# robertteleng/aria-slam

Measured on AMD Instinct MI355X. Metric: frames/s ORB extract+BF-match, 640x480 @2000 kp, higher is better.
Workload: dtype u8

## Files before the change

### aria_slam_amd/csrc/fast_blur_stream.hip

```cpp
#include <hip/hip_runtime.h>

#include <algorithm>
#include <cstdint>
#include <cstdio>
#include <cstdlib>

#include "common.h"
#include "orb_device.h"
#include "orb_kernels.h"

namespace aria {

namespace {

constexpr int kRing = 16;
#ifndef ARIA_STREAM_PEND_LDS
#define ARIA_STREAM_PEND_LDS 1
#endif
constexpr int kQ1 = 256;
constexpr int kQ2 = 512;
#ifndef ARIA_STREAM_COMPACT_LDS
#define ARIA_STREAM_COMPACT_LDS 1
#endif
#if ARIA_STREAM_COMPACT_LDS
// ... 776 lines not shown
                const uint8_t* rowb = s_rawb + roff(rb);
                const bool reuse = oy == hprev_row;
                uint32_t qb0[4], qb1[4], qa0[4] = {0, 0, 0, 0}, qa1[4] = {0, 0, 0, 0};
#pragma unroll
                for (int i = 0; i < 4; i++) {
                    const uint32_t* qb = reinterpret_cast<const uint32_t*>(rowb + xo[i]);
                    qb0[i] = qb[0]; qb1[i] = qb[1];
                }
                if (!reuse) {
#pragma unroll
                    for (int i = 0; i < 4; i++) {
                        const uint32_t* qa = reinterpret_cast<const uint32_t*>(rowa + xo[i]);
                        qa0[i] = qa[0]; qa1[i] = qa[1];
                    }
                }
                uint32_t outw = 0;
#pragma unroll
                for (int i = 0; i < 4; i++) {
                    const us2v wx = __builtin_bit_cast(us2v, xw[i]);
                    uint32_t h0 = hprev[i];
                    if (!reuse) h0 = __builtin_amdgcn_udot2(__builtin_bit_cast(us2v, __builtin_amdgcn_perm(qa1[i], qa0[i], xs[i])), wx, 0u, false);
                    const uint32_t bot = __builtin_amdgcn_perm(qb1[i], qb0[i], xs[i]);
                    const uint32_t h1 = __builtin_amdgcn_udot2(__builtin_bit_cast(us2v, bot), wx, 0u, false);
                    const uint32_t v = __builtin_amdgcn_udot2(__builtin_bit_cast(us2v, h0 | (h1 << 16)), __builtin_bit_cast(us2v, cyp), 32768u, false);
                    outw = __builtin_amdgcn_perm(v, outw, put[i]);
                    hprev[i] = h1;
                }
                gstore_sv<uint32_t>(next0 + (int64_t)dy_next * A.next_pitch, nout_off, outw);
            }
            hprev_row = rb;
            dy_next++;
        }
        wave_sync();
    };
    for (int gi = 0; gi < G; gi += 2) {
        group(b0, gi);
        group(b1, gi + 1);
    }
}

#ifndef ARIA_STREAM_WAVES4
#define ARIA_STREAM_WAVES4 1
#endif
#if ARIA_STREAM_WAVES4
static_assert(ARIA_STREAM_COMPACT_LDS, "four waves per SIMD need the 10 240-byte LDS layout");
#define ARIA_STREAM_OCC __attribute__((amdgpu_waves_per_eu(4, 4)))
#else
#define ARIA_STREAM_OCC
#endif
template <int WPB>
__global__ __launch_bounds__(64 * WPB) ARIA_STREAM_OCC void k_fast_blur_stream(StreamArgs A, unsigned long long* __restrict__ stamps) {
    extern __shared__ __attribute__((aligned(16))) uint8_t smem[];
    const int lane = threadIdx.x & 63;
    const int wv = __builtin_amdgcn_readfirstlane((int)(threadIdx.x >> 6));
    const int w = A.w, h = A.h;
    const int D = (w + 3) >> 2, U = D + 2;
    int wave_id = (int)blockIdx.x * WPB + wv;
    bool role_pyr = false;
    if (ARIA_STREAM_SPLIT && A.next != nullptr) {
        role_pyr = (((wave_id >> 3) ^ __popc(wave_id >> 4)) & 1) != 0;
        wave_id = ((wave_id >> 4) << 3) | (wave_id & 7);
    }
    const int per_seg = 8 * A.panels8;
    const int seg = wave_id / per_seg, rr = wave_id - seg * per_seg;
    const int pw = (rr & 7) * A.panels8 + (rr >> 3);
    if (seg >= A.n_seg || pw >= A.panels) return;
    const int64_t total = (int64_t)A.n_frames * U;
    const int64_t pos0 = (int64_t)pw * kOwned - 1;
    int64_t pos = pos0 + lane;
    const bool valid = pos >= 0 && pos < total;
    pos = min(max(pos, (int64_t)0), total - 1);
    LaneRole R;
    R.frame = (int)(pos / U);
    const int j = (int)(pos - (int64_t)R.frame * U);
    R.gdw = j - 1;
    const int frame0 = __builtin_amdgcn_readfirstlane(R.frame);
    const int r4 = w & 3;
    if (R.gdw < 0 || R.gdw >= D) R.sel = 0x00010203u;
    else if (r4 && R.gdw == D - 1) R.sel = r4 == 1 ? 0x00010203u : r4 == 2 ? 0x01020302u : 0x02030201u;
    else R.sel = 0x03020100u;
    const bool data = valid && R.gdw >= 0 && R.gdw < D;
    R.owner = data && lane >= 1 && lane <= kOwned;
    const bool level_has_kp = (w > 2 * kEdgeThreshold) && (h > 2 * kEdgeThreshold);
    const int fx0 = kEdgeThreshold - 1, fx1 = w - kEdgeThreshold;
    R.xm0 = R.xm1 = 0;
    R.tailbits = 0;
    if (data) {
        const int x = 4 * R.gdw;
#pragma unroll
        for (int i = 0; i < 4; i++) {
            const bool scored = (lane >= 1 && lane <= kOwned) || (lane == 0 && i == 3) || (lane == 63 && i == 0);
            if (level_has_kp && scored && x + i >= fx0 && x + i <= fx1) {
                if (i < 2) R.xm0 |= (i & 1) ? 0x80000000u : 0x00008000u;
                else R.xm1 |= (i & 1) ? 0x80000000u : 0x00008000u;
            }
            if (x + i >= A.tail_start) R.tailbits |= 1u << i;
        }
    }
    uint8_t* wl = smem + wv * kWaveLds;
    const bool any_tail = __builtin_amdgcn_ballot_w64(R.tailbits != 0) != 0;
#if ARIA_STREAM_SPLIT
#ifdef ARIA_PROBE_SPLIT_EMPTY_PYR
    if (role_pyr) return;
#endif
    if (role_pyr) pyramid_wave(A, wl, lane, R, frame0, seg);
    else if (any_tail) stream_wave<WPB, true, true, false>(A, wl, lane, R, frame0, seg, stamps);
    else stream_wave<WPB, false, true, false>(A, wl, lane, R, frame0, seg, stamps);
#else
    (void)role_pyr;
#if ARIA_STREAM_PYR_INWALK
    if (A.next == nullptr) {
        if (any_tail) stream_wave<WPB, true, true, false>(A, wl, lane, R, frame0, seg, stamps);
        else stream_wave<WPB, false, true, false>(A, wl, lane, R, frame0, seg, stamps);
        return;
    }
#endif
    if (any_tail) stream_wave<WPB, true, true, true>(A, wl, lane, R, frame0, seg, stamps);
    else stream_wave<WPB, false, true, true>(A, wl, lane, R, frame0, seg, stamps);
#endif
}

bool stream_eligible(const Plan& P, const FrameSrc& S) {
    (void)S;
    for (int l = 0; l < kLevels; l++)
        if (P.lv[l].w < 16 || P.lv[l].h < 16) return false;
    return P.stream_ok != 0;
}

int stream_set_attributes() {
    ARIA_HIP(hipFuncSetAttribute(reinterpret_cast<const void*>(k_fast_blur_stream<1>), hipFuncAttributeMaxDynamicSharedMemorySize, 160 * 1024 - 64));
    ARIA_HIP(hipFuncSetAttribute(reinterpret_cast<const void*>(k_fast_blur_stream<2>), hipFuncAttributeMaxDynamicSharedMemorySize, 160 * 1024 - 64));
    ARIA_HIP(hipFuncSetAttribute(reinterpret_cast<const void*>(k_fast_blur_stream<4>), hipFuncAttributeMaxDynamicSharedMemorySize, 160 * 1024 - 64));
    return ARIA_OK;
}

int blur_tail_start(int tie_mode, int w) {
    switch (tie_mode) {
        case 0: return 0;
        case 2: return w & ~7;
        case 3: return w & ~15;
        default: return w & ~3;
    }
}

void launch_fast_blur_stream(const Plan& P, const FrameSrc& S, const DeviceScratch& D, int n_frames, hipStream_t st,
                             Profiler* prof, LaunchCtx& ctx) {
#ifdef ARIA_DIAG
    static const bool want_stamps = [] { const char* e = aria_getenv("ARIA_STREAM_STAMPS"); return e && e[0] == '1'; }();
#else
    const bool want_stamps = false;
#endif
    static unsigned long long* d_stamps = nullptr;
    if (want_stamps && !d_stamps) hipMalloc(&d_stamps, 8 * sizeof(unsigned long long));
    (void)ctx;
    static const int seg_force = [] { const char* e = aria_getenv("ARIA_STREAM_SEG_ROWS"); return e ? atoi(e) : 0; }();
    static const int wpb = [] { const char* e = aria_getenv("ARIA_STREAM_WPB"); const int v = e ? atoi(e) : 1; return (v == 2 || v == 4) ? v : 1; }();
    for (int l = 0; l < kLevels; l++) {
        const LevelGeom& g = P.lv[l];
        const int U = ((g.w + 3) >> 2) + 2;
        const int64_t total = (int64_t)n_frames * U;
        const int64_t panels = (total + kOwned - 1) / kOwned;
        int n_seg = (int)std::min<int64_t>(std::max<int64_t>((6 * 256 * 12 + panels - 1) / panels, 1), std::max(g.h / 64, 1));
        if (seg_force > 0) n_seg = std::min(std::max(g.h / seg_force, 1), 64);
        const int seg_rows = ((g.h + n_seg - 1) / n_seg + 3) & ~3;
        n_seg = (g.h + seg_rows - 1) / seg_rows;
        const int64_t panels8 = (panels + 7) / 8;
        const int64_t waves = 8 * panels8 * n_seg * ((ARIA_STREAM_SPLIT && l + 1 < kLevels) ? 2 : 1);
        const dim3 grid((unsigned)((waves + wpb - 1) / wpb));
        StreamArgs A{};
        A.seg_rows = seg_rows; A.n_seg = n_seg; A.panels = (int)panels; A.panels8 = (int)panels8;
        if (l == 0) { A.src = S.img; A.src_fstride = S.frame_stride; A.src_pitch = S.row_stride; }
        else { A.src = D.raw + g.raw_off; A.src_fstride = P.raw_frame_bytes; A.src_pitch = g.pitch; }
        A.blur = D.blur + g.blur_off; A.blur_fstride = P.blur_frame_bytes; A.blur_pitch = g.pitch;
        A.cand = D.cand + g.cand_off; A.cand_fstride = P.cand_frame_entries; A.cand_cap = g.cand_cap;
        A.cand_cnt = D.cand_cnt + l; A.err = D.err;
        A.w = g.w; A.h = g.h; A.n_frames = n_frames; A.thr = P.fast_threshold; A.tail_start = blur_tail_start(P.tie_mode, g.w);
        if (l + 1 < kLevels) {
            const LevelGeom& gn = P.lv[l + 1];
            A.next = D.raw + gn.raw_off; A.next_fstride = P.raw_frame_bytes; A.next_pitch = gn.pitch; A.next_w = gn.w; A.next_h = gn.h;
            A.xt = D.tab + gn.xtab; A.yt = D.tab + gn.ytab; A.xinv = D.tab + gn.xinv; A.ytr = D.tab + gn.ytr;
        } else {
            A.ytr = D.tab + P.lv[1].ytr;
        }
        static const size_t lds_pad = [] { const char* e = aria_getenv("ARIA_STREAM_LDS_KB"); return e ? (size_t)atoi(e) * 1024 : (size_t)0; }();
#define ARIA_FS_LAUNCH(N) ARIA_LAUNCH(prof, (k_fast_blur_stream<N>), grid, dim3(64 * N), std::max((size_t)N * kWaveLds, lds_pad), st, A, d_stamps)
        if (d_stamps) hipMemsetAsync(d_stamps, 0, 8 * sizeof(unsigned long long), st);
        if (wpb == 1) ARIA_FS_LAUNCH(1); else if (wpb == 2) ARIA_FS_LAUNCH(2); else ARIA_FS_LAUNCH(4);
#undef ARIA_FS_LAUNCH
        if (d_stamps) {
            hipStreamSynchronize(st);
            unsigned long long hs[8];
            hipMemcpy(hs, d_stamps, sizeof(hs), hipMemcpyDeviceToHost);
            const double n = (double)std::max(1ull, hs[7]);
            fprintf(stderr, "[stream stamps L%d] %llu waves, ticks per wave: ring %.0f walk %.0f append+score %.0f rows-in %.0f nms+emit %.0f pyramid %.0f\n",
                    l, hs[7], hs[0] / n, hs[1] / n, hs[2] / n, hs[5] / n, hs[3] / n, hs[4] / n);
        }
    }
}

}
```

### aria_slam_amd/csrc/orb_kernels.h

```cpp
#pragma once
#include <hip/hip_runtime.h>
#include <hip/hip_ext.h>

#include <cstdint>
#include <vector>

#include "aria_orb_hip.h"
#include "orb_plan.h"

namespace aria {

struct FrameSrc {
    const uint8_t* img;
    int64_t frame_stride;
    int row_stride;
    int aligned4;
    int aligned16;
};

struct DeviceScratch {
    uint8_t* raw;
    uint8_t* blur;
    uint32_t* cand;
    int* cand_cnt;
    uint4* sel;
    int* sel_cnt;
    uint32_t* tab;
    int* pyr_bands;
    int* err;
    int* ovf;
    int2* ovf_items;
    unsigned long long* ovf_keys;
    long long ovf_keys_cap;
    uint4* osel;
    int osel_cap;
};

enum { STAGE_RESIZE = 0, STAGE_FAST_BLUR = 1, STAGE_SELECT = 2, STAGE_DESCRIBE = 3, STAGE_COUNT = 4 };
struct LaunchEvents { hipEvent_t start, stop; int stage; int launches; };
struct Profiler {
    bool enabled = false;
    unsigned stage_mask = ~0u;
    bool open = false;
    std::vector<LaunchEvents> pending;
    std::vector<hipEvent_t> pool;
    double ms[STAGE_COUNT] = {0, 0, 0, 0};
    int64_t launches[STAGE_COUNT] = {0, 0, 0, 0};
    int64_t frames = 0;
    LaunchEvents cur{};
    hipEvent_t get();
    void begin(int stage, hipStream_t st);
    void count() { cur.launches++; }
    void end(hipStream_t st);
    void collect();
    void release();
};

struct EnvConfig {
    int ablate;
    int level_streams;
    int stamp_level;
    int sel_stamps;
    int band_trim;
    int band_xcd_map;
    int select_bitonic;
    int desc_stamps;
    int desc_quad;
    int fast_blur_impl;
    int fuse_resize;
    int pyr_impl;
    int rs_impl;
    int band_budget_kb, band_qpct0, band_qstep;
    int batch_stream;
};
const EnvConfig& env_config();

struct LaunchCtx {
    int device = -1;
    int schedule = 0;
    int* hdr = nullptr;
    const uint8_t* host_img = nullptr;
    hipEvent_t stage_event[4] = {};
    bool stage_events_armed = false;
    bool last_blur_q4 = false;
    const char* last_fast_blur = "";
    hipStream_t side[kLevels] = {};
    hipEvent_t ev_fork = nullptr, ev_join[kLevels] = {}, ev_lvl[kLevels] = {};
    unsigned long long* d_band_stamps = nullptr;
    unsigned long long* d_sel_stamps = nullptr;
    unsigned long long* d_desc_stamps = nullptr;
    int init(int device);
    void release();
};

#define ARIA_LAUNCH(prof, kernel, grid, block, lds, st, ...)                       \
    do {                                                                           \
        if ((prof) && (prof)->open) (prof)->count();                               \
        hipLaunchKernelGGL(kernel, grid, block, lds, st, __VA_ARGS__);             \
    } while (0)

void launch_fast_blur_band(const Plan& P, const FrameSrc& S, const DeviceScratch& D, int n_frames, hipStream_t st,
                           Profiler* prof, bool fuse_resize, LaunchCtx& ctx);
void launch_band2(const Plan& P, const FrameSrc& S, const DeviceScratch& D, int n_frames, hipStream_t st, Profiler* prof,
                  bool fuse_resize, LaunchCtx& ctx);
int band2_set_attributes();
void launch_fast_blur_stream(const Plan& P, const FrameSrc& S, const DeviceScratch& D, int n_frames, hipStream_t st,
                             Profiler* prof, LaunchCtx& ctx);
bool stream_eligible(const Plan& P, const FrameSrc& S);
int stream_set_attributes();
int blur_tail_start(int tie_mode, int w);
int band_set_attributes();
int band_init_ctx(LaunchCtx& ctx);
int band_side_streams(LaunchCtx& ctx);

struct BandAll { int first[kLevels + 1]; int qcap[kLevels]; int xcd_map; int lpr[kLevels]; };
bool launch_pyramid_fused(const Plan& P, const FrameSrc& S, const DeviceScratch& D, int n_frames, hipStream_t st, Profiler* prof,
                          int* clr_a = nullptr, int n_a = 0, int* clr_b = nullptr, int n_b = 0,
                          const uint8_t* src_alt = nullptr, uint8_t* copy_dst = nullptr);
bool pyramid_fused_available(const Plan& P);
bool latency_zero_copy(const Plan& P, const LaunchCtx& ctx, const Profiler* prof);
void launch_pyramid_level(const Plan& P, const FrameSrc& S, const DeviceScratch& D, int n_frames, hipStream_t st, Profiler* prof, int l);
void launch_pyramid_and_band_latency(const Plan& P, const FrameSrc& S, const DeviceScratch& D, int n_frames, hipStream_t st,
                                     Profiler* prof, LaunchCtx& ctx);
void launch_pyramid_pass(const Plan& P, const FrameSrc& S, const DeviceScratch& D, int n_frames, hipStream_t st, Profiler* prof);
int pyramid_set_attributes();
void launch_fast_blur_tile(const Plan& P, const FrameSrc& S, const DeviceScratch& D, int n_frames, hipStream_t st, Profiler* prof);

void launch_extract_chunk(const Plan& P, const FrameSrc& S, const DeviceScratch& D, int n_frames,
                          aria_keypoint* d_kps, uint8_t* d_desc, int* d_counts, int kp_cap, hipStream_t st,
                          Profiler* prof, LaunchCtx& ctx);

}
```

### aria_slam_amd/csrc/orb_kernels.hip

```cpp
#include <hip/hip_runtime.h>

#include <cfloat>
#include <cstdint>
#include <cstdlib>

#include "common.h"
#include "orb_device.h"
#include "orb_kernels.h"

namespace aria {

struct PatternLaneMajor { uint32_t w[16][16]; };
constexpr PatternLaneMajor make_pattern_lane_major() {
    constexpr int src[1024] = {
#include "orb_pattern_31.inc"
    };
    PatternLaneMajor p{};
    for (int l = 0; l < 16; l++)
        for (int it = 0; it < 16; it++) {
            const int t = 16 * it + l;
            p.w[l][it] = ((uint32_t)(src[4 * t] & 0xFF)) | ((uint32_t)(src[4 * t + 1] & 0xFF) << 8) |
                         ((uint32_t)(src[4 * t + 2] & 0xFF) << 16) | ((uint32_t)(src[4 * t + 3] & 0xFF) << 24);
        }
    return p;
}
__device__ __attribute__((aligned(16))) const PatternLaneMajor kPattern31 = make_pattern_lane_major();

#define ARIA_UMAX_LIST {15, 15, 15, 15, 14, 14, 14, 13, 13, 12, 11, 10, 9, 8, 6, 3}

struct IcMaskLaneMajor { uint32_t m[16][16]; };
constexpr IcMaskLaneMajor make_ic_mask() {
    constexpr int umax[16] = ARIA_UMAX_LIST;
    IcMaskLaneMajor t{};
    for (int l = 0; l < 16; l++)
        for (int k = 0; k < 16; k++) {
            const int r = 2 * k + (l >> 3), j = l & 7;
            uint32_t w = 0;
            for (int b = 0; b < 4 && r < 31; b++) {
                const int u = 4 * j + b - 15, v = r - 15;
                const int au = u < 0 ? -u : u, av = v < 0 ? -v : v;
                if (au <= 15 && au <= umax[av]) w |= 0xFFu << (8 * b);
            }
            t.m[l][k] = w;
        }
    return t;
}
__device__ __attribute__((aligned(16))) const IcMaskLaneMajor kIcMask = make_ic_mask();

typedef short s2v __attribute__((ext_vector_type(2)));
__device__ __forceinline__ void harris_row_pairs(const uint8_t* rowp, int xs, int sh, bool dword_ok, uint32_t* E) {
    uint32_t w0, w1, w2;
    if (dword_ok) {
        const uint32_t* q = reinterpret_cast<const uint32_t*>(rowp + xs);
        w0 = q[0]; w1 = q[1]; w2 = q[2];
    } else {
        const uint8_t* q = rowp + xs;
        w0 = (uint32_t)q[0] | ((uint32_t)q[1] << 8) | ((uint32_t)q[2] << 16) | ((uint32_t)q[3] << 24);
        w1 = (uint32_t)q[4] | ((uint32_t)q[5] << 8) | ((uint32_t)q[6] << 16) | ((uint32_t)q[7] << 24);
        w2 = (uint32_t)q[8] | ((uint32_t)q[9] << 8) | ((uint32_t)q[10] << 16) | ((uint32_t)q[11] << 24);
    }
    const uint32_t a = __builtin_amdgcn_alignbyte(w1, w0, (uint32_t)sh);
    const uint32_t b = __builtin_amdgcn_alignbyte(w2, w1, (uint32_t)sh);
    E[0] = __builtin_amdgcn_perm(0u, a, 0x0c010c00u);
    E[1] = __builtin_amdgcn_perm(0u, a, 0x0c030c02u);
    E[2] = __builtin_amdgcn_perm(0u, b, 0x0c010c00u);
    E[3] = __builtin_amdgcn_perm(0u, b, 0x0c030c02u);
    E[4] = (w2 >> (8 * sh)) & 0xFFu;
}

__device__ __forceinline__ uint32_t pk16_add(uint32_t a, uint32_t b) {
    return __builtin_bit_cast(uint32_t, __builtin_bit_cast(s2v, a) + __builtin_bit_cast(s2v, b));
}
__device__ __forceinline__ uint32_t pk16_sub(uint32_t a, uint32_t b) {
    return __builtin_bit_cast(uint32_t, __builtin_bit_cast(s2v, a) - __builtin_bit_cast(s2v, b));
}

__device__ __forceinline__ float harris_response(const uint8_t* img, int pitch, int x, int y, bool dword_ok) {
    int a = 0, b = 0, c = 0;
    const int xs = (x - 4) & ~3, sh = (x - 4) & 3;
    const uint8_t* base = img + (int64_t)(y - 4) * pitch;
    uint32_t R[9][5];
#pragma unroll
    for (int r = 0; r < 9; r++) harris_row_pairs(base + (int64_t)r * pitch, xs, sh, dword_ok, R[r]);
#pragma unroll
    for (int i = 1; i <= 7; i++) {
        uint32_t sE[5], dE[5];
#pragma unroll
        for (int k = 0; k < 5; k++) {
            sE[k] = pk16_add(pk16_add(R[i - 1][k], R[i + 1][k]), pk16_add(R[i][k], R[i][k]));
            dE[k] = pk16_sub(R[i + 1][k], R[i - 1][k]);
        }
#pragma unroll
        for (int k = 0; k < 4; k++) {
            uint32_t ix = pk16_sub(sE[k + 1], sE[k]);
            const uint32_t dO = __builtin_amdgcn_alignbit(dE[k + 1], dE[k], 16);
            uint32_t iy = pk16_add(pk16_add(dE[k], dE[k + 1]), pk16_add(dO, dO));
            if (k == 3) { ix &= 0xFFFFu; iy &= 0xFFFFu; }
            const s2v vx = __builtin_bit_cast(s2v, ix), vy = __builtin_bit_cast(s2v, iy);
            a = __builtin_amdgcn_sdot2(vx, vx, a, false);
            b = __builtin_amdgcn_sdot2(vy, vy, b, false);
            c = __builtin_amdgcn_sdot2(vx, vy, c, false);
        }
    }
    const float scale = 1.f / ((1 << 2) * 7 * 255.f);
    const float scale_sq_sq = scale * scale * scale * scale;
    const float k = 0.04f;
    return ((float)a * (float)b - (float)c * (float)c - k * ((float)a + (float)b) * ((float)a + (float)b)) * scale_sq_sq;
}

__device__ void select_ovf_item(const Plan& P, const FrameSrc& S, const uint8_t* __restrict__ raw,
                                const uint32_t* __restrict__ cand, const int* __restrict__ cand_cnt,
                                uint4* __restrict__ sel, int* __restrict__ sel_cnt, int* __restrict__ err,
                                int* __restrict__ ovf, unsigned long long* __restrict__ keys, long long keys_cap,
                                uint4* __restrict__ osel, int osel_cap, int frame, int l, int* s_hist, int* s_misc);

template <bool INLINE_OVF, int NT>
__global__ __launch_bounds__(NT) void k_select(Plan P, FrameSrc S, const uint8_t* __restrict__ raw,
                                                const uint32_t* __restrict__ cand, const int* __restrict__ cand_cnt,
                                                uint4* __restrict__ sel, int* __restrict__ sel_cnt,
                                                int* __restrict__ err, unsigned long long* __restrict__ stamps,
                                                int* __restrict__ ovf, int2* __restrict__ ovf_items,
                                                unsigned long long* __restrict__ ovf_keys, long long ovf_keys_cap,
                                                uint4* __restrict__ osel, int osel_cap, int force_bitonic) {
    static_assert(kLevels == 8, "level rotation below assumes 8 levels");
    const int l = (int)((blockIdx.x + blockIdx.y) & 7u), frame = blockIdx.y;
#define SSTAMP(k) do { if (stamps && threadIdx.x == 0) stamps[((size_t)blockIdx.y * kLevels + l) * 8 + (k)] = __builtin_amdgcn_s_memtime(); } while (0)
    SSTAMP(0);
    extern __shared__ __attribute__((aligned(16))) unsigned long long s_keys[];
    __shared__ int s_hist[256];
    __shared__ int s_misc[4];
    __shared__ int s_wsum[NT / 64];
    __shared__ int s_bin[1024];

    const int tid = threadIdx.x;
    const bool lead = tid < 256;
    const LevelGeom g = P.lv[l];
    const uint32_t* clist = cand + (int64_t)frame * P.cand_frame_entries + g.cand_off;
    const int n = min(cand_cnt[frame * kLevels + l], g.cand_cap);
    const int q = g.quota;
    const int kSortCap = P.sort_cap;

    if (q == 0 || n == 0) {
        if (tid == 0) sel_cnt[frame * kLevels + l] = 0;
        return;
    }
    if (lead) s_hist[tid] = 0;
    if (tid == 0) { s_misc[1] = 0; s_misc[2] = 0; }
    __syncthreads();
    constexpr int kUnroll = 8;
    for (int i0 = 0; i0 < n; i0 += NT * kUnroll) {
        uint32_t v[kUnroll];
#pragma unroll
        for (int u = 0; u < kUnroll; u++) {
            const int i = i0 + u * NT + tid;
            v[u] = i < n ? clist[i] : 0u;
        }
#pragma unroll
        for (int u = 0; u < kUnroll; u++)
            if (i0 + u * NT + tid < n) atomicAdd(&s_hist[v[u] >> 22], 1);
    }
    __syncthreads();
    SSTAMP(1);
    {
        const int lane = tid & 63, wv = tid >> 6;
        int c = s_hist[255 - (tid & 255)];
#pragma unroll
        for (int d = 1; d < 64; d <<= 1) {
            const int o = __shfl_up(c, d);
            if (lane >= d) c += o;
        }
        if (lane == 63) s_wsum[wv] = c;
        if (tid == 0) s_misc[0] = 0;
        __syncthreads();
        int before = 0;
#pragma unroll
        for (int w = 0; w < 3; w++)
            if (w < wv) before += s_wsum[w];
        const int cum = c + before;
        const int own = s_hist[255 - (tid & 255)];
        if (lead && n > 2 * q && cum >= 2 * q && cum - own < 2 * q) s_misc[0] = 255 - tid;
        __syncthreads();
    }
    const int thr = s_misc[0];
    for (int i0 = 0; i0 < n; i0 += NT * kUnroll) {
        uint32_t v[kUnroll];
#pragma unroll
        for (int u = 0; u < kUnroll; u++) {
            const int i = i0 + u * NT + tid;
            v[u] = i < n ? clist[i] : 0u;
        }
#pragma unroll
        for (int u = 0; u < kUnroll; u++) {
            const bool keep = i0 + u * NT + tid < n && (int)(v[u] >> 22) >= thr;
            const unsigned long long m = __ballot(keep);
            if (m) {
                const int lane = tid & 63, leader = __ffsll((long long)m) - 1;
                int base = 0;
                if (lane == leader) base = atomicAdd(&s_misc[1], __popcll(m));
                base = __shfl(base, leader);
                const int slot = base + __popcll(m & ((1ull << lane) - 1ull));
                if (keep && slot < kSortCap) s_keys[slot] = (unsigned long long)v[u];
            }
        }
    }
    __syncthreads();
    SSTAMP(2);
    int pitch;
    const uint8_t* img = raw_level_ptr(P, S, raw, frame, l, pitch);
    {
        const int ns = min(s_misc[1], kSortCap);
        for (int i = tid; i < ns; i += NT) {
            const uint32_t cd = (uint32_t)s_keys[i];
            const int x = cd & 0x7FF, y = (cd >> 11) & 0x7FF;
            const float r = harris_response(img, pitch, x, y, (l > 0) || S.aligned4);
            uint32_t u = __float_as_uint(r);
            u = (u & 0x80000000u) ? ~u : (u | 0x80000000u);
            s_keys[i] = ((unsigned long long)(~u) << 32) | ((uint32_t)y << 16) | (uint32_t)x;
        }
    }
    __syncthreads();
    SSTAMP(3);
    int n1 = s_misc[1];
    if (n1 > kSortCap) {
        if (INLINE_OVF) {
            __shared__ __attribute__((aligned(8))) int s_ovm[8];
            if (!lead) return;
            select_ovf_item(P, S, raw, cand, cand_cnt, sel, sel_cnt, err, ovf, ovf_keys, ovf_keys_cap, osel, osel_cap, frame, l,
                            s_hist, s_ovm);
            return;
        }
        if (tid == 0) {
            sel_cnt[frame * kLevels + l] = 0;
            const int it = atomicAdd(&ovf[0], 1);
            if (it < kOvfItems) ovf_items[it] = make_int2(frame, l);
            else atomicOr(err, ERRBIT_SORT_OVERFLOW);
        }
        return;
    }
    __shared__ int s_srt[2];
    auto hbin = [](unsigned long long kk) { return (int)min((uint32_t)(kk >> 53), 1023u); };
    const bool cut = n1 > q + 64;
    for (int i = tid; i < 1024; i += NT) s_bin[i] = 0;
    if (tid == 0) { s_srt[0] = 1023; s_srt[1] = 0; }
    __syncthreads();
    for (int i = tid; i < n1; i += NT) atomicAdd(&s_bin[hbin(s_keys[i])], 1);
    __syncthreads();
    {
        const int lane = tid & 63, wv = tid >> 6;
        int b[4], tot = 0;
#pragma unroll
        for (int k = 0; k < 4; k++) { b[k] = lead ? s_bin[4 * tid + k] : 0; tot += b[k]; }
        int c = tot;
#pragma unroll
        for (int d = 1; d < 64; d <<= 1) {
            const int o = __shfl_up(c, d);
            if (lane >= d) c += o;
        }
        if (lane == 63) s_wsum[wv] = c;
        if (tid == 0) s_misc[1] = 0;
        __syncthreads();
        int run = c - tot;
#pragma unroll
        for (int w = 0; w < 3; w++)
            if (w < wv) run += s_wsum[w];
#pragma unroll
        for (int k = 0; k < 4; k++) {
            if (lead) s_bin[4 * tid + k] = run;
            if (lead && cut && run < q && run + b[k] >= q) s_srt[0] = 4 * tid + k;
            run += b[k];
        }
        __syncthreads();
        const int bc = s_srt[0];
        int mx = 0;
#pragma unroll
        for (int k = 0; k < 4; k++)
            if (lead && 4 * tid + k <= bc) mx = max(mx, b[k]);
        if (mx > 0) atomicMax(&s_srt[1], mx);
    }
// ... 804 lines not shown
#pragma unroll
            for (int k = 0; k < 7; k++) {
                const int row = (5 * k + 5 < 31) ? 5 * k + rr : min(5 * k + rr, 30);
                rv[k] = *reinterpret_cast<const DwordQuad*>(gp + row * p64);
            }
        } else {
#pragma unroll
            for (int k = 0; k < 7; k++) {
                const int row = (5 * k + 5 < 31) ? 5 * k + rr : min(5 * k + rr, 30);
                const uint8_t* q = gp + row * p64;
                rv[k].a = (uint32_t)q[0] | ((uint32_t)q[1] << 8) | ((uint32_t)q[2] << 16) | ((uint32_t)q[3] << 24);
                rv[k].b = (uint32_t)q[4] | ((uint32_t)q[5] << 8) | ((uint32_t)q[6] << 16) | ((uint32_t)q[7] << 24);
                rv[k].c = (uint32_t)q[8] | ((uint32_t)q[9] << 8) | ((uint32_t)q[10] << 16) | ((uint32_t)q[11] << 24);
                rv[k].d = (uint32_t)q[12] | ((uint32_t)q[13] << 8) | ((uint32_t)q[14] << 16) | ((uint32_t)q[15] << 24);
            }
        }
#pragma unroll
        for (int k = 0; k < 7; k++) {
            const int row = (5 * k + 5 < 31) ? 5 * k + rr : min(5 * k + rr, 30);
            *reinterpret_cast<uint4*>(sr + row * kIcPitch) = make_uint4(rv[k].a, rv[k].b, rv[k].c, rv[k].d);
        }
    }
    if (stamps) { asm volatile("s_waitcnt vmcnt(0) lgkmcnt(0)" ::: "memory"); }
    DSTAMP(2);
    __builtin_amdgcn_wave_barrier();

    const int sh = (x - xr) - kHalfPatch;
    const int hp = l16 >> 3, jj = l16 & 7;
    const uint8_t* rbase = s_raw[wv * 4 + grp] + 4 * jj + (sh & ~3);
    const uint32_t wu = 0x04030201u + 0x04040404u * (uint32_t)jj;
    uint32_t acc_u = 0, acc_v = 0, acc_s = 0;
#pragma unroll
    for (int k = 0; k < 16; k++) {
        const int r = min(2 * k + hp, 30);
        const uint32_t lo = *reinterpret_cast<const uint32_t*>(rbase + r * kIcPitch);
        const uint32_t hi = *reinterpret_cast<const uint32_t*>(rbase + r * kIcPitch + 4);
        const uint32_t pix = __builtin_amdgcn_alignbyte(hi, lo, sh) & icm[k];
        acc_u = __builtin_amdgcn_udot4(pix, wu, acc_u, false);
        acc_v = __builtin_amdgcn_udot4(pix, 0x01010101u * (uint32_t)(2 * k + 1), acc_v, false);
        acc_s = __builtin_amdgcn_sad_u8(pix, 0u, acc_s);
    }
    const int sum_u = row16_sum((int)acc_u), sum_v = row16_sum((int)acc_v);
    const int s_half = row8_sum((int)acc_s);
    const int s_othr = __builtin_amdgcn_update_dpp(0, s_half, 0x140, 0xF, 0xF, true);
    const int s_all = s_half + s_othr;
    const int s_hp1 = hp ? s_half : s_othr;
    const int m10 = sum_u - 16 * s_all;
    const int m01 = sum_v + s_hp1 - 16 * s_all;
    const float angle = fast_atan2_deg((float)m01, (float)m10);
    DSTAMP(3);

    float ang = angle;
    ang *= (float)(3.1415926535897932384626433832795 / 180.f);
    double sd, cd;
    det_sincos((double)ang, sd, cd);
    const float a = (float)cd, b = (float)sd;
    __builtin_amdgcn_wave_barrier();
    constexpr int kPitchL = Q4 ? kDescPitchQ : kDescPitch;
    if constexpr (Q4) {
        uint8_t* sp = s_patch[wv * 4 + grp];
#pragma unroll
        for (int k = 0; k < kPv; k++) {
            uint32_t* d = reinterpret_cast<uint32_t*>(sp + (4 * pq[k]) * kPitchL + 4 * pc[k]);
            d[0] = pv[k].a; d[kPitchL / 4] = pv[k].b; d[2 * kPitchL / 4] = pv[k].c; d[3 * kPitchL / 4] = pv[k].d;
        }
    } else {
        const int r4 = l16 >> 2, c4 = l16 & 3;
        uint8_t* sp = s_patch[wv * 4 + grp] + 16 * c4;
#pragma unroll
        for (int k = 0; k < 10; k++) {
            const int row = (4 * k + 4 <= kDescRows) ? 4 * k + r4 : min(4 * k + r4, kDescRows - 1);
            *reinterpret_cast<uint4*>(sp + row * kDescPitch) = make_uint4(pv[k].a, pv[k].b, pv[k].c, pv[k].d);
        }
    }
    const uint8_t* bc = s_patch[wv * 4 + grp] + (y - ys) * kPitchL + (x - xs);
    __builtin_amdgcn_wave_barrier();
    typedef float f2 __attribute__((ext_vector_type(2)));
    const f2 aa = {a, a}, bb = {b, b}, nbb = {-b, -b};
    const f2 magic = {12582912.0f, 12582912.0f};
    constexpr uint32_t kMagicBits = 0x4B400000u;
    const uint8_t* bc0 = bc - (size_t)(0x400000u * (uint32_t)kPitchL + kMagicBits);
    DSTAMP(4);
    uint32_t mine = 0;
#pragma unroll
    for (int it = 0; it < 16; it++) {
        const float px0 = (float)(signed char)(pat[it] & 0xFF), py0 = (float)(signed char)((pat[it] >> 8) & 0xFF);
        const float px1 = (float)(signed char)((pat[it] >> 16) & 0xFF), py1 = (float)(signed char)((pat[it] >> 24) & 0xFF);
        const f2 PX = {px0, px1}, PY = {py0, py1};
        const f2 fx = PX * aa + PY * nbb + magic;
        const f2 fy = PX * bb + PY * aa + magic;
        const uint32_t o0 = __umul24(__float_as_uint(fy.x), kPitchL) + __float_as_uint(fx.x);
        const uint32_t o1 = __umul24(__float_as_uint(fy.y), kPitchL) + __float_as_uint(fx.y);
        const int t0 = bc0[o0];
        const int t1 = bc0[o1];
        const unsigned long long m = __ballot(t0 < t1);
        if (__builtin_amdgcn_inverse_ballot_w64(0x0001000100010001ull << it)) mine = (uint32_t)(m >> (16 * grp)) & 0xFFFFu;
    }
    DSTAMP(5);
    if (valid && fits) {
        const int64_t orow = (int64_t)frame * kp_cap + oidx;
        *reinterpret_cast<uint16_t*>(desc + orow * 32 + 2 * l16) = (uint16_t)mine;
        if (l16 == 0) {
            aria_keypoint k;
            k.x = (float)x * g.scale;
            k.y = (float)y * g.scale;
            k.size = kPatchSize * g.scale;
            k.angle = angle;
            k.response = __uint_as_float(sv.y);
            k.octave = l;
            kps[orow] = k;
        }
    }
    };
    if constexpr (MODE == 0) {
        describe_block((int)blockIdx.x, false);
    } else if constexpr (MODE == 1) {
        const int n_blk = (min(ovf[1], osel_cap) + kDescKp - 1) / kDescKp;
        for (int blk = blockIdx.x; blk < n_blk; blk += gridDim.x) describe_block(blk, true);
    } else {
        if ((int)blockIdx.x < n_regular) {
            describe_block((int)blockIdx.x, false);
        } else {
            const int n_blk = (min(ovf[1], osel_cap) + kDescKp - 1) / kDescKp;
            for (int blk = (int)blockIdx.x - n_regular; blk < n_blk; blk += kDescArenaBlocks) describe_block(blk, true);
        }
    }
    DSTAMP(6);
#undef DSTAMP
}

static int env_int(const char* name, int dflt) { const char* e = aria_getenv(name); return e ? atoi(e) : dflt; }
static bool env_is(const char* name, char c) { const char* e = aria_getenv(name); return e && e[0] == c; }

const EnvConfig& env_config() {
    static const EnvConfig cfg = [] {
        EnvConfig c{};
        c.ablate = env_int("ARIA_ABLATE", 0);
        c.level_streams = env_is("ARIA_LEVEL_STREAMS", '1') ? 1 : 0;
        c.stamp_level = env_int("ARIA_STAMPS", -1);
        c.sel_stamps = env_is("ARIA_SEL_STAMPS", '1') ? 1 : 0;
        c.select_bitonic = env_is("ARIA_SELECT_SORT", 'b') ? 1 : 0;
        c.band_xcd_map = env_is("ARIA_BAND_XCD_MAP", '0') ? 0 : 1;
        c.band_trim = env_is("ARIA_BAND_TRIM", '0') ? 0 : 1;
        c.desc_stamps = env_is("ARIA_DESC_STAMPS", '1') ? 1 : 0;
        c.desc_quad = env_is("ARIA_DESC_IMPL", 'q') ? 1 : 0;
        c.fast_blur_impl = env_is("ARIA_FAST_BLUR_IMPL", 't') ? 0 : env_is("ARIA_FAST_BLUR_IMPL", 'm') ? 1 : 2;
        c.pyr_impl = env_is("ARIA_PYRAMID_IMPL", 'f') ? 1 : 0;
        c.rs_impl = env_is("ARIA_RESIZE_IMPL", 'd') ? 0 : env_is("ARIA_RESIZE_IMPL", 'l') ? 1 : 2;
        c.fuse_resize = (c.fast_blur_impl != 0 && !env_is("ARIA_RESIZE_FUSE", '0') && !aria_getenv("ARIA_RESIZE_IMPL") &&
                         !aria_getenv("ARIA_PYRAMID_IMPL") && !c.level_streams) ? 1 : 0;
        c.band_budget_kb = env_int("ARIA_BAND_BUDGET_KB", 0);
        c.band_qpct0 = env_int("ARIA_BAND_QPCT0", -1);
        c.band_qstep = env_int("ARIA_BAND_QPCT_STEP", -1);
        c.batch_stream = (c.fast_blur_impl == 2 && !env_is("ARIA_FAST_BLUR_IMPL", 'b') && c.fuse_resize && c.stamp_level < 0) ? 1 : 0;
        return c;
    }();
    return cfg;
}

hipEvent_t Profiler::get() {
    if (!pool.empty()) { hipEvent_t e = pool.back(); pool.pop_back(); return e; }
    hipEvent_t e = nullptr;
    if (hipEventCreate(&e) != hipSuccess) return nullptr;
    return e;
}
void Profiler::begin(int stage, hipStream_t st) {
    open = enabled && ((stage_mask >> stage) & 1u);
    if (!open) return;
    cur = LaunchEvents{get(), get(), stage, 0};
    hipStreamSynchronize(st);
    hipEventRecord(cur.start, st);
}
void Profiler::end(hipStream_t st) {
    if (!open) return;
    open = false;
    hipEventRecord(cur.stop, st);
    hipStreamSynchronize(st);
    pending.push_back(cur);
}
void Profiler::collect() {
    for (LaunchEvents& le : pending) {
        float t = 0.f;
        if (hipEventElapsedTime(&t, le.start, le.stop) == hipSuccess) ms[le.stage] += t;
        launches[le.stage] += le.launches;
        pool.push_back(le.start);
        pool.push_back(le.stop);
    }
    pending.clear();
}
void Profiler::release() {
    collect();
    for (hipEvent_t e : pool) hipEventDestroy(e);
    pool.clear();
}

int LaunchCtx::init(int dev) {
    device = dev;
    const EnvConfig& E = env_config();
    ARIA_HIP(hipFuncSetAttribute(reinterpret_cast<const void*>(k_select<false, 256>), hipFuncAttributeMaxDynamicSharedMemorySize,
                                 (int)(sizeof(unsigned long long) * kSortCapMax)));
    ARIA_HIP(hipFuncSetAttribute(reinterpret_cast<const void*>(k_select<true, 256>), hipFuncAttributeMaxDynamicSharedMemorySize,
                                 (int)(sizeof(unsigned long long) * kSortCapMax)));
    if (int prc = pyramid_set_attributes(); prc != ARIA_OK) return prc;
    int rc = band_set_attributes();
    if (rc != ARIA_OK) return rc;
#ifdef ARIA_VARIANTS
    rc = band2_set_attributes();
    if (rc != ARIA_OK) return rc;
#endif
    rc = stream_set_attributes();
    if (rc != ARIA_OK) return rc;
    rc = band_init_ctx(*this);
    if (rc != ARIA_OK) return rc;
    if (E.sel_stamps) ARIA_HIP(hipMalloc(&d_sel_stamps, sizeof(unsigned long long) * 8 * kLevels * 4096));
    if (E.desc_stamps) ARIA_HIP(hipMalloc(&d_desc_stamps, sizeof(unsigned long long) * 8 * (1u << 22)));
    return ARIA_OK;
}

void LaunchCtx::release() {
    for (int l = 0; l < kLevels; l++) {
        if (side[l]) hipStreamDestroy(side[l]);
        if (ev_join[l]) hipEventDestroy(ev_join[l]);
        if (ev_lvl[l]) hipEventDestroy(ev_lvl[l]);
        side[l] = nullptr; ev_join[l] = nullptr; ev_lvl[l] = nullptr;
    }
    if (ev_fork) hipEventDestroy(ev_fork);
    ev_fork = nullptr;
    hipFree(d_band_stamps); hipFree(d_sel_stamps); hipFree(d_desc_stamps);
    d_band_stamps = d_sel_stamps = d_desc_stamps = nullptr;
}

static bool latency_schedule(const LaunchCtx& ctx, const Profiler* prof) {
    return ctx.schedule == 1 && ctx.ev_fork != nullptr && env_config().fast_blur_impl == 2 && !(prof && prof->enabled);
}

bool latency_zero_copy(const Plan& P, const LaunchCtx& ctx, const Profiler* prof) {
    static const bool off = [] { const char* e = aria_getenv("ARIA_ZERO_COPY"); return !(e && e[0] == '1'); }();
    const char* f = aria_getenv("ARIA_LATENCY_FORK");
    return !off && !(f && f[0] == '1') && ctx.host_img != nullptr && latency_schedule(ctx, prof) && pyramid_fused_available(P);
}

void launch_extract_chunk(const Plan& P, const FrameSrc& S, const DeviceScratch& D, int n_frames,
                          aria_keypoint* d_kps, uint8_t* d_desc, int* d_counts, int kp_cap, hipStream_t st,
                          Profiler* prof, LaunchCtx& ctx) {
    const EnvConfig& E = env_config();
    if (prof && prof->enabled) prof->frames += n_frames;

    const bool latency = latency_schedule(ctx, prof);
    const bool fuse_resize = E.fuse_resize != 0 && !latency;
    ctx.last_blur_q4 = false;
    if (!latency) {
        hipMemsetAsync(D.ovf, 0, sizeof(int) * (4 + kLevels * (size_t)n_frames), st);
        if (ctx.hdr) hipMemsetAsync(ctx.hdr, 0, 64, st);
    }
    if (latency) {
        ctx.last_fast_blur = "k_fast_blur_band";
        launch_pyramid_and_band_latency(P, S, D, n_frames, st, prof, ctx);
    } else {
#ifdef ARIA_VARIANTS
    if (!fuse_resize) {
        if (prof) prof->begin(STAGE_RESIZE, st);
        launch_pyramid_pass(P, S, D, n_frames, st, prof);
        if (prof) prof->end(st);
    }
#endif

    if (prof) prof->begin(STAGE_FAST_BLUR, st);
    if (E.batch_stream && fuse_resize && stream_eligible(P, S)) {
        ctx.last_fast_blur = "k_fast_blur_stream";
        ctx.last_blur_q4 = true;
        launch_fast_blur_stream(P, S, D, n_frames, st, prof, ctx);
#ifdef ARIA_VARIANTS
    } else if (E.fast_blur_impl == 1 && !E.level_streams && P.tie_mode <= 1) {
        ctx.last_fast_blur = "k_band2";
        launch_band2(P, S, D, n_frames, st, prof, fuse_resize, ctx);
    } else if (E.fast_blur_impl == 0 && P.tie_mode <= 1) {
        ctx.last_fast_blur = "k_fast_blur";
        launch_fast_blur_tile(P, S, D, n_frames, st, prof);
#endif
    } else {
        ctx.last_fast_blur = "k_fast_blur_band";
        launch_fast_blur_band(P, S, D, n_frames, st, prof, fuse_resize, ctx);
    }
    if (prof) prof->end(st);
    }

    if (ctx.stage_events_armed && ctx.stage_event[STAGE_SELECT]) hipEventRecord(ctx.stage_event[STAGE_SELECT], st);
    if (prof) prof->begin(STAGE_SELECT, st);
    unsigned long long* sstp = (ctx.d_sel_stamps && n_frames <= 4096) ? ctx.d_sel_stamps : nullptr;
    if (sstp) hipMemsetAsync(sstp, 0, sizeof(unsigned long long) * 8 * kLevels * (size_t)n_frames, st);
    if (latency)
        ARIA_LAUNCH(prof, (k_select<true, 256>), dim3(kLevels, n_frames), dim3(256), sizeof(unsigned long long) * (size_t)P.sort_cap,
                    st, P, S, D.raw, D.cand, D.cand_cnt, D.sel, D.sel_cnt, D.err, sstp, D.ovf, D.ovf_items, D.ovf_keys,
                    D.ovf_keys_cap, D.osel, D.osel_cap, E.select_bitonic);
    else
        ARIA_LAUNCH(prof, (k_select<false, 256>), dim3(kLevels, n_frames), dim3(256), sizeof(unsigned long long) * (size_t)P.sort_cap,
                    st, P, S, D.raw, D.cand, D.cand_cnt, D.sel, D.sel_cnt, D.err, sstp, D.ovf, D.ovf_items, D.ovf_keys,
                    D.ovf_keys_cap, D.osel, D.osel_cap, E.select_bitonic);
    if (!latency)
    ARIA_LAUNCH(prof, k_select_ovf, dim3(64), dim3(256), 0, st, P, S, D.raw, D.cand, D.cand_cnt, D.sel, D.sel_cnt, D.err,
                D.ovf, D.ovf_items, D.ovf_keys, D.ovf_keys_cap, D.osel, D.osel_cap);
    if (sstp) {
        hipStreamSynchronize(st);
        std::vector<unsigned long long> hs((size_t)n_frames * kLevels * 8);
        hipMemcpy(hs.data(), sstp, hs.size() * 8, hipMemcpyDeviceToHost);
        for (int l = 0; l < kLevels; l += 7) {
            double ph[5] = {0}; int n = 0;
            for (int f = 0; f < n_frames; f++) {
                const unsigned long long* q = &hs[((size_t)f * kLevels + l) * 8];
                if (!q[5]) continue;
                for (int k = 0; k < 5; k++) ph[k] += (double)(q[k + 1] - q[k]);
                n++;
            }
            if (n) fprintf(stderr, "[select stamps L%d] %d blocks, cycles: hist %.0f cut+compact %.0f harris %.0f sort %.0f emit %.0f\n",
                           l, n, ph[0] / n, ph[1] / n, ph[2] / n, ph[3] / n, ph[4] / n);
        }
    }

    if (prof) prof->end(st);

    if (prof) prof->begin(STAGE_DESCRIBE, st);
    {
        const bool w16 = !latency && ctx.last_blur_q4 && !E.desc_quad;
        const int bpf = w16 ? (desc16_waves_per_frame(P) + kDescWaves - 1) / kDescWaves : (P.sel_frame_entries + kDescKp - 1) / kDescKp;
        const int frames8 = (n_frames + 7) / 8 * 8;
        const size_t nwaves = (size_t)bpf * frames8 * kDescWaves;
        unsigned long long* stp = (ctx.d_desc_stamps && nwaves <= (1u << 22)) ? ctx.d_desc_stamps : nullptr;
        if (stp) hipMemsetAsync(stp, 0, sizeof(unsigned long long) * 8 * nwaves, st);
        if (latency) {
            ARIA_LAUNCH(prof, (k_describe<2, false>), dim3((unsigned)(bpf * frames8 + kDescArenaBlocks)), dim3(64 * kDescWaves), 0, st, P, S,
                        D.raw, D.blur, D.sel, D.sel_cnt, d_kps, d_desc, d_counts, kp_cap, D.err, n_frames, bpf, stp,
                        (const uint4*)D.osel, (const int*)D.ovf, D.osel_cap);
        } else if (w16) {
            ARIA_LAUNCH(prof, (k_describe<0, true, true>), dim3((unsigned)(bpf * frames8)), dim3(64 * kDescWaves), 0, st, P, S, D.raw,
                        D.blur, D.sel, D.sel_cnt, d_kps, d_desc, d_counts, kp_cap, D.err, n_frames, bpf, stp, (const uint4*)nullptr,
                        (const int*)nullptr, 0);
            ARIA_LAUNCH(prof, (k_describe<1, true, true>), dim3(256), dim3(64 * kDescWaves), 0, st, P, S,
                        D.raw, D.blur, D.sel, D.sel_cnt, d_kps, d_desc, d_counts, kp_cap, D.err, n_frames, bpf,
                        (unsigned long long*)nullptr, (const uint4*)D.osel, (const int*)D.ovf, D.osel_cap);
#ifdef ARIA_VARIANTS
        } else if (ctx.last_blur_q4) {
            ARIA_LAUNCH(prof, (k_describe<0, true>), dim3((unsigned)(bpf * frames8)), dim3(64 * kDescWaves), 0, st, P, S, D.raw, D.blur,
                        D.sel, D.sel_cnt, d_kps, d_desc, d_counts, kp_cap, D.err, n_frames, bpf, stp, (const uint4*)nullptr,
                        (const int*)nullptr, 0);
            ARIA_LAUNCH(prof, (k_describe<1, true>), dim3(256), dim3(64 * kDescWaves), 0, st, P, S,
                        D.raw, D.blur, D.sel, D.sel_cnt, d_kps, d_desc, d_counts, kp_cap, D.err, n_frames, bpf,
                        (unsigned long long*)nullptr, (const uint4*)D.osel, (const int*)D.ovf, D.osel_cap);
#endif
        } else {
            ARIA_LAUNCH(prof, (k_describe<0, false>), dim3((unsigned)(bpf * frames8)), dim3(64 * kDescWaves), 0, st, P, S, D.raw, D.blur,
                        D.sel, D.sel_cnt, d_kps, d_desc, d_counts, kp_cap, D.err, n_frames, bpf, stp, (const uint4*)nullptr,
                        (const int*)nullptr, 0);
            ARIA_LAUNCH(prof, (k_describe<1, false>), dim3(256), dim3(64 * kDescWaves), 0, st, P, S,
                        D.raw, D.blur, D.sel, D.sel_cnt, d_kps, d_desc, d_counts, kp_cap, D.err, n_frames, bpf,
                        (unsigned long long*)nullptr, (const uint4*)D.osel, (const int*)D.ovf, D.osel_cap);
        }
        if (stp) {
            hipStreamSynchronize(st);
            std::vector<unsigned long long> hs(nwaves * 8);
            hipMemcpy(hs.data(), stp, hs.size() * 8, hipMemcpyDeviceToHost);
            double ph[6] = {0}; size_t n = 0;
            const int np = w16 ? 5 : 6;
            for (size_t w = 0; w < nwaves; w++) {
                if (!hs[w * 8 + np] || !hs[w * 8 + 1]) continue;
                if (!w16 && !hs[w * 8 + 5]) continue;
                for (int k = 0; k < np; k++) ph[k] += (double)(hs[w * 8 + k + 1] - hs[w * 8 + k]);
                n++;
            }
            if (n && w16)
                fprintf(stderr, "[describe stamps] 16-kp form, %zu waves, 100 MHz ticks: sel %.1f moment rounds %.1f atan+sincos %.1f pattern rounds %.1f records %.1f\n",
                        n, ph[0] / n, ph[1] / n, ph[2] / n, ph[3] / n, ph[4] / n);
            else if (n)
                fprintf(stderr, "[describe stamps] %zu waves, 100 MHz ticks: sel %.1f windows %.1f moments+atan %.1f sincos %.1f pattern %.1f store %.1f\n",
                        n, ph[0] / n, ph[1] / n, ph[2] / n, ph[3] / n, ph[4] / n, ph[5] / n);
        }
    }
    if (prof) prof->end(st);
}

}
```

Measured before the change: 389,400.

## Overlap per-level select kernels with streaming FAST/blur on a side stream

After each pyramid level's fast-blur-stream kernel, an event is recorded and that level's select kernel is launched on a separate stream, so selection for finished levels runs concurrently with FAST/blur of later levels. The main stream joins on the side stream before the overflow pass instead of launching one monolithic select over all levels. The select kernel gains a level argument to pin the block to one level. This adds event and stream overhead and splits select into eight smaller launches, which could under-fill the GPU for small batches, and a higher-priority stream is available behind an environment flag.

```diff
diff --git a/aria_slam_amd/csrc/fast_blur_stream.hip b/aria_slam_amd/csrc/fast_blur_stream.hip
--- a/aria_slam_amd/csrc/fast_blur_stream.hip
+++ b/aria_slam_amd/csrc/fast_blur_stream.hip
@@ -952,7 +952,6 @@
 #endif
     static unsigned long long* d_stamps = nullptr;
     if (want_stamps && !d_stamps) hipMalloc(&d_stamps, 8 * sizeof(unsigned long long));
-    (void)ctx;
     static const int seg_force = [] { const char* e = aria_getenv("ARIA_STREAM_SEG_ROWS"); return e ? atoi(e) : 0; }();
     static const int wpb = [] { const char* e = aria_getenv("ARIA_STREAM_WPB"); const int v = e ? atoi(e) : 1; return (v == 2 || v == 4) ? v : 1; }();
     for (int l = 0; l < kLevels; l++) {
@@ -987,6 +986,7 @@
         if (d_stamps) hipMemsetAsync(d_stamps, 0, 8 * sizeof(unsigned long long), st);
         if (wpb == 1) ARIA_FS_LAUNCH(1); else if (wpb == 2) ARIA_FS_LAUNCH(2); else ARIA_FS_LAUNCH(4);
 #undef ARIA_FS_LAUNCH
+        if (ctx.select_overlap && !d_stamps) launch_select_level(P, S, D, n_frames, l, st, ctx);
         if (d_stamps) {
             hipStreamSynchronize(st);
             unsigned long long hs[8];
diff --git a/aria_slam_amd/csrc/orb_kernels.h b/aria_slam_amd/csrc/orb_kernels.h
--- a/aria_slam_amd/csrc/orb_kernels.h
+++ b/aria_slam_amd/csrc/orb_kernels.h
@@ -72,6 +72,7 @@
     int rs_impl;
     int band_budget_kb, band_qpct0, band_qstep;
     int batch_stream;
+    int select_prio;
 };
 const EnvConfig& env_config();
 
@@ -86,6 +87,11 @@
     const char* last_fast_blur = "";
     hipStream_t side[kLevels] = {};
     hipEvent_t ev_fork = nullptr, ev_join[kLevels] = {}, ev_lvl[kLevels] = {};
+    hipStream_t sel_stream = nullptr;
+    hipEvent_t sel_ev_lvl[kLevels] = {}, sel_ev_join = nullptr;
+    bool sel_streams_failed = false;
+    bool select_overlap = false;
+    int sel_levels_launched = 0;
     unsigned long long* d_band_stamps = nullptr;
     unsigned long long* d_sel_stamps = nullptr;
     unsigned long long* d_desc_stamps = nullptr;
@@ -106,6 +112,7 @@
 int band2_set_attributes();
 void launch_fast_blur_stream(const Plan& P, const FrameSrc& S, const DeviceScratch& D, int n_frames, hipStream_t st,
                              Profiler* prof, LaunchCtx& ctx);
+void launch_select_level(const Plan& P, const FrameSrc& S, const DeviceScratch& D, int n_frames, int l, hipStream_t st, LaunchCtx& ctx);
 bool stream_eligible(const Plan& P, const FrameSrc& S);
 int stream_set_attributes();
 int blur_tail_start(int tie_mode, int w);
diff --git a/aria_slam_amd/csrc/orb_kernels.hip b/aria_slam_amd/csrc/orb_kernels.hip
--- a/aria_slam_amd/csrc/orb_kernels.hip
+++ b/aria_slam_amd/csrc/orb_kernels.hip
@@ -121,9 +121,9 @@
                                                 int* __restrict__ err, unsigned long long* __restrict__ stamps,
                                                 int* __restrict__ ovf, int2* __restrict__ ovf_items,
                                                 unsigned long long* __restrict__ ovf_keys, long long ovf_keys_cap,
-                                                uint4* __restrict__ osel, int osel_cap, int force_bitonic) {
+                                                uint4* __restrict__ osel, int osel_cap, int force_bitonic, int level) {
     static_assert(kLevels == 8, "level rotation below assumes 8 levels");
-    const int l = (int)((blockIdx.x + blockIdx.y) & 7u), frame = blockIdx.y;
+    const int l = (int)((level >= 0 ? (unsigned)level : blockIdx.x + blockIdx.y) & 7u), frame = blockIdx.y;
 #define SSTAMP(k) do { if (stamps && threadIdx.x == 0) stamps[((size_t)blockIdx.y * kLevels + l) * 8 + (k)] = __builtin_amdgcn_s_memtime(); } while (0)
     SSTAMP(0);
     extern __shared__ __attribute__((aligned(16))) unsigned long long s_keys[];
@@ -1234,6 +1234,7 @@
         c.band_budget_kb = env_int("ARIA_BAND_BUDGET_KB", 0);
         c.band_qpct0 = env_int("ARIA_BAND_QPCT0", -1);
         c.band_qstep = env_int("ARIA_BAND_QPCT_STEP", -1);
+        c.select_prio = env_is("ARIA_SELECT_PRIO", 'h') ? 1 : 0;
         c.batch_stream = (c.fast_blur_impl == 2 && !env_is("ARIA_FAST_BLUR_IMPL", 'b') && c.fuse_resize && c.stamp_level < 0) ? 1 : 0;
         return c;
     }();
@@ -1308,6 +1309,13 @@
     }
     if (ev_fork) hipEventDestroy(ev_fork);
     ev_fork = nullptr;
+    if (sel_stream) hipStreamDestroy(sel_stream);
+    if (sel_ev_join) hipEventDestroy(sel_ev_join);
+    sel_stream = nullptr; sel_ev_join = nullptr;
+    for (int l = 0; l < kLevels; l++) {
+        if (sel_ev_lvl[l]) hipEventDestroy(sel_ev_lvl[l]);
+        sel_ev_lvl[l] = nullptr;
+    }
     hipFree(d_band_stamps); hipFree(d_sel_stamps); hipFree(d_desc_stamps);
     d_band_stamps = d_sel_stamps = d_desc_stamps = nullptr;
 }
@@ -1320,6 +1328,38 @@
     static const bool off = [] { const char* e = aria_getenv("ARIA_ZERO_COPY"); return !(e && e[0] == '1'); }();
     const char* f = aria_getenv("ARIA_LATENCY_FORK");
     return !off && !(f && f[0] == '1') && ctx.host_img != nullptr && latency_schedule(ctx, prof) && pyramid_fused_available(P);
+}
+
+constexpr int kSelectOverlapMinFrames = 64;
+
+static int select_overlap_streams(LaunchCtx& ctx) {
+    if (ctx.sel_stream) return ARIA_OK;
+    if (env_config().select_prio) {
+        int lo = 0, hi = 0;
+        ARIA_HIP(hipDeviceGetStreamPriorityRange(&lo, &hi));
+        ARIA_HIP(hipStreamCreateWithPriority(&ctx.sel_stream, hipStreamNonBlocking, hi));
+    } else {
+        ARIA_HIP(create_stream(&ctx.sel_stream));
+    }
+    ARIA_HIP(hipEventCreateWithFlags(&ctx.sel_ev_join, hipEventDisableTiming));
+    for (int l = 0; l < kLevels; l++) ARIA_HIP(hipEventCreateWithFlags(&ctx.sel_ev_lvl[l], hipEventDisableTiming));
+    return ARIA_OK;
+}
+
+static bool select_overlap_wanted(const LaunchCtx& ctx, const Profiler* prof, int n_frames) {
+    if (prof && prof->enabled && ((prof->stage_mask >> STAGE_SELECT) & 1u)) return false;
+    if (ctx.d_sel_stamps || ctx.sel_streams_failed) return false;
+    if (env_is("ARIA_SELECT_OVERLAP", '0')) return false;
+    return n_frames >= env_int("ARIA_SELECT_OVERLAP_MIN", kSelectOverlapMinFrames);
+}
+
+void launch_select_level(const Plan& P, const FrameSrc& S, const DeviceScratch& D, int n_frames, int l, hipStream_t st, LaunchCtx& ctx) {
+    hipEventRecord(ctx.sel_ev_lvl[l], st);
+    hipStreamWaitEvent(ctx.sel_stream, ctx.sel_ev_lvl[l], 0);
+    hipLaunchKernelGGL((k_select<false, 256>), dim3(1, n_frames), dim3(256), sizeof(unsigned long long) * (size_t)P.sort_cap,
+                       ctx.sel_stream, P, S, D.raw, D.cand, D.cand_cnt, D.sel, D.sel_cnt, D.err, (unsigned long long*)nullptr, D.ovf,
+                       D.ovf_items, D.ovf_keys, D.ovf_keys_cap, D.osel, D.osel_cap, env_config().select_bitonic, l);
+    ctx.sel_levels_launched++;
 }
 
 void launch_extract_chunk(const Plan& P, const FrameSrc& S, const DeviceScratch& D, int n_frames,
@@ -1331,6 +1371,7 @@
     const bool latency = latency_schedule(ctx, prof);
     const bool fuse_resize = E.fuse_resize != 0 && !latency;
     ctx.last_blur_q4 = false;
+    ctx.sel_levels_launched = 0;
     if (!latency) {
         hipMemsetAsync(D.ovf, 0, sizeof(int) * (4 + kLevels * (size_t)n_frames), st);
         if (ctx.hdr) hipMemsetAsync(ctx.hdr, 0, 64, st);
@@ -1351,7 +1392,10 @@
     if (E.batch_stream && fuse_resize && stream_eligible(P, S)) {
         ctx.last_fast_blur = "k_fast_blur_stream";
         ctx.last_blur_q4 = true;
+        ctx.select_overlap = select_overlap_wanted(ctx, prof, n_frames);
+        if (ctx.select_overlap && select_overlap_streams(ctx) != ARIA_OK) ctx.select_overlap = false, ctx.sel_streams_failed = true;
         launch_fast_blur_stream(P, S, D, n_frames, st, prof, ctx);
+        ctx.select_overlap = false;
 #ifdef ARIA_VARIANTS
     } else if (E.fast_blur_impl == 1 && !E.level_streams && P.tie_mode <= 1) {
         ctx.last_fast_blur = "k_band2";
@@ -1371,14 +1415,18 @@
     if (prof) prof->begin(STAGE_SELECT, st);
     unsigned long long* sstp = (ctx.d_sel_stamps && n_frames <= 4096) ? ctx.d_sel_stamps : nullptr;
     if (sstp) hipMemsetAsync(sstp, 0, sizeof(unsigned long long) * 8 * kLevels * (size_t)n_frames, st);
-    if (latency)
+    const bool sel_done = ctx.sel_levels_launched == kLevels;
+    if (sel_done) {
+        hipEventRecord(ctx.sel_ev_join, ctx.sel_stream);
+        hipStreamWaitEvent(st, ctx.sel_ev_join, 0);
+    } else if (latency)
         ARIA_LAUNCH(prof, (k_select<true, 256>), dim3(kLevels, n_frames), dim3(256), sizeof(unsigned long long) * (size_t)P.sort_cap,
                     st, P, S, D.raw, D.cand, D.cand_cnt, D.sel, D.sel_cnt, D.err, sstp, D.ovf, D.ovf_items, D.ovf_keys,
-                    D.ovf_keys_cap, D.osel, D.osel_cap, E.select_bitonic);
+                    D.ovf_keys_cap, D.osel, D.osel_cap, E.select_bitonic, -1);
     else
         ARIA_LAUNCH(prof, (k_select<false, 256>), dim3(kLevels, n_frames), dim3(256), sizeof(unsigned long long) * (size_t)P.sort_cap,
                     st, P, S, D.raw, D.cand, D.cand_cnt, D.sel, D.sel_cnt, D.err, sstp, D.ovf, D.ovf_items, D.ovf_keys,
-                    D.ovf_keys_cap, D.osel, D.osel_cap, E.select_bitonic);
+                    D.ovf_keys_cap, D.osel, D.osel_cap, E.select_bitonic, -1);
     if (!latency)
     ARIA_LAUNCH(prof, k_select_ovf, dim3(64), dim3(256), 0, st, P, S, D.raw, D.cand, D.cand_cnt, D.sel, D.sel_cnt, D.err,
                 D.ovf, D.ovf_items, D.ovf_keys, D.ovf_keys_cap, D.osel, D.osel_cap);
```

After: 384,400. 1.3% lower.
